# theteamatx/x-edr-trajectory-planning

Measured on AMD Instinct MI355X. Metric: time-optimal path timings/s (7-DOF, 2000 s-samples), 1/2/4/8 MI355X + %HBM roofline, higher is better.
Workload: dtype f64

## Files before the change

x-edr-trajectory-planning_amd/csrc/tpamd_sweep_joint.h:

```cpp
#pragma once

#include <type_traits>

#include "tpamd_kernels.h"

namespace tpamd {

__device__ __forceinline__ double uniform_f64(double v) {
  const int lo = __builtin_amdgcn_readfirstlane(__double2loint(v));
  const int hi = __builtin_amdgcn_readfirstlane(__double2hiint(v));
  return __hiloint2double(hi, lo);
}
__device__ __forceinline__ double readlane_f64(double v, int lane) {
  const int lo = __builtin_amdgcn_readlane(__double2loint(v), lane);
  const int hi = __builtin_amdgcn_readlane(__double2hiint(v), lane);
  return __hiloint2double(hi, lo);
}
__device__ __forceinline__ int uniform_i32(int v) { return __builtin_amdgcn_readfirstlane(v); }

template <int CTRL>
__device__ __forceinline__ double dpp_f64(double v) {
  int lo = __double2loint(v), hi = __double2hiint(v);
  lo = __builtin_amdgcn_update_dpp(0, lo, CTRL, 0xf, 0xf, true);
  hi = __builtin_amdgcn_update_dpp(0, hi, CTRL, 0xf, 0xf, true);
  return __hiloint2double(hi, lo);
}

template <bool MAX>
__device__ __forceinline__ double ext2_raw(double a, double b) {
  double r;
  if (MAX) asm("v_max_f64 %0, %1, %2" : "=v"(r) : "v"(a), "v"(b));
  else asm("v_min_f64 %0, %1, %2" : "=v"(r) : "v"(a), "v"(b));
  return r;
}

template <bool MAX>
__device__ __forceinline__ double row16_extreme(double v) {
  double o;
  o = dpp_f64<0xB1>(v);  v = ext2_raw<MAX>(o, v);
  o = dpp_f64<0x4E>(v);  v = ext2_raw<MAX>(o, v);
  o = dpp_f64<0x141>(v); v = ext2_raw<MAX>(o, v);
  o = dpp_f64<0x140>(v); v = ext2_raw<MAX>(o, v);
  return v;
}

#define TPAMD_OS_STEP(HALF, C)                                                            \
  "s_mov_b32 exec_" HALF ", %[m" #C "]\n\t"                                               \
  "v_fmac_f64_dpp %[acc], %[d], %[one] row_newbcast:" #C " row_mask:0xf bank_mask:0xf\n\t"
#define TPAMD_OS_ROW(HALF, OTHER)                                                                      \
  asm volatile("s_mov_b64 %[sv], exec\n\ts_mov_b32 exec_" OTHER ", 0\n\t"                              \
               TPAMD_OS_STEP(HALF, 0) TPAMD_OS_STEP(HALF, 1) TPAMD_OS_STEP(HALF, 2) TPAMD_OS_STEP(HALF, 3)     \
               TPAMD_OS_STEP(HALF, 4) TPAMD_OS_STEP(HALF, 5) TPAMD_OS_STEP(HALF, 6) TPAMD_OS_STEP(HALF, 7)     \
               TPAMD_OS_STEP(HALF, 8) TPAMD_OS_STEP(HALF, 9) TPAMD_OS_STEP(HALF, 10) TPAMD_OS_STEP(HALF, 11)   \
               TPAMD_OS_STEP(HALF, 12) TPAMD_OS_STEP(HALF, 13) TPAMD_OS_STEP(HALF, 14) TPAMD_OS_STEP(HALF, 15) \
               "s_mov_b64 exec, %[sv]\n\t"                                                             \
               : [acc] "+v"(acc), [sv] "=&s"(save)                                                     \
               : [d] "v"(d), [one] "v"(one), TPAMD_OS_M(0), TPAMD_OS_M(1), TPAMD_OS_M(2), TPAMD_OS_M(3), \
                 TPAMD_OS_M(4), TPAMD_OS_M(5), TPAMD_OS_M(6), TPAMD_OS_M(7), TPAMD_OS_M(8), TPAMD_OS_M(9), \
                 TPAMD_OS_M(10), TPAMD_OS_M(11), TPAMD_OS_M(12), TPAMD_OS_M(13), TPAMD_OS_M(14), TPAMD_OS_M(15))
template <int ROW>
__device__ __forceinline__ void ordered_sum_row(double &acc, double d, double one) {
  constexpr unsigned SH = (ROW & 1) ? 16u : 0u;
#define TPAMD_OS_M(C) [m##C] "n"((int)(((0xffffu << C) & 0xffffu) << SH))
  unsigned long long save;
  if (ROW < 2) TPAMD_OS_ROW("lo", "hi");
  else TPAMD_OS_ROW("hi", "lo");
#undef TPAMD_OS_M
}
template <int ROW>
__device__ __forceinline__ void ordered_sum_carry(double &acc) {
  int lo = __double2loint(acc), hi = __double2hiint(acc);
  lo = __builtin_amdgcn_update_dpp(lo, lo, 0x142, 1 << ROW, 0xf, false);
  hi = __builtin_amdgcn_update_dpp(hi, hi, 0x142, 1 << ROW, 0xf, false);
  acc = __hiloint2double(hi, lo);
}
__device__ __forceinline__ double ordered_sum64(double t, double d) {
  double acc = t;
  const double one = 1.0;
  ordered_sum_row<0>(acc, d, one);
  ordered_sum_carry<1>(acc);
  ordered_sum_row<1>(acc, d, one);
  ordered_sum_carry<2>(acc);
  ordered_sum_row<2>(acc, d, one);
  ordered_sum_carry<3>(acc);
  ordered_sum_row<3>(acc, d, one);
  return acc;
}

struct OrderedSumMasks {
  double m[15];
  __device__ __forceinline__ void init(int lane) {
#pragma unroll
    for (int c = 1; c < 16; c++) m[c - 1] = ((lane & 15) >= c) ? 1.0 : 0.0;
  }
};
#define TPAMD_OSM_STEP(C, ROWMASK)                                                                    \
  "v_fmac_f64_dpp %[acc], %[d], %[m" #C "] row_newbcast:" #C " row_mask:" ROWMASK " bank_mask:0xf\n\t"
#define TPAMD_OSM_ROW(ROWMASK)                                                                          \
  asm volatile(TPAMD_OSM_STEP(0, ROWMASK) TPAMD_OSM_STEP(1, ROWMASK) TPAMD_OSM_STEP(2, ROWMASK)         \
               TPAMD_OSM_STEP(3, ROWMASK) TPAMD_OSM_STEP(4, ROWMASK) TPAMD_OSM_STEP(5, ROWMASK)         \
               TPAMD_OSM_STEP(6, ROWMASK) TPAMD_OSM_STEP(7, ROWMASK) TPAMD_OSM_STEP(8, ROWMASK)         \
               TPAMD_OSM_STEP(9, ROWMASK) TPAMD_OSM_STEP(10, ROWMASK) TPAMD_OSM_STEP(11, ROWMASK)       \
               TPAMD_OSM_STEP(12, ROWMASK) TPAMD_OSM_STEP(13, ROWMASK) TPAMD_OSM_STEP(14, ROWMASK)      \
               TPAMD_OSM_STEP(15, ROWMASK)                                                              \
               : [acc] "+v"(acc)                                                                        \
               : [d] "v"(d), [m0] "v"(one), [m1] "v"(k.m[0]), [m2] "v"(k.m[1]), [m3] "v"(k.m[2]),       \
                 [m4] "v"(k.m[3]), [m5] "v"(k.m[4]), [m6] "v"(k.m[5]), [m7] "v"(k.m[6]), [m8] "v"(k.m[7]), \
                 [m9] "v"(k.m[8]), [m10] "v"(k.m[9]), [m11] "v"(k.m[10]), [m12] "v"(k.m[11]),           \
                 [m13] "v"(k.m[12]), [m14] "v"(k.m[13]), [m15] "v"(k.m[14]))
__device__ __forceinline__ double ordered_sum64_finite(double t, double d, const OrderedSumMasks &k) {
  double acc = t;
  const double one = 1.0;
  asm volatile("s_nop 1" ::: "memory");
  TPAMD_OSM_ROW("0x1");
  ordered_sum_carry<1>(acc);
  TPAMD_OSM_ROW("0x2");
  ordered_sum_carry<2>(acc);
  TPAMD_OSM_ROW("0x4");
  ordered_sum_carry<3>(acc);
  TPAMD_OSM_ROW("0x8");
  return acc;
}

#ifdef TPAMD_DIAG
__device__ __forceinline__ long long tpamd_stamp() {
  unsigned long long t;
  __builtin_amdgcn_sched_barrier(0);
  asm volatile("s_memtime %0\n\ts_waitcnt lgkmcnt(0)" : "=s"(t)::"memory");
  __builtin_amdgcn_sched_barrier(0);
  return (long long)t;
}
#define TPAMD_T0(var) const long long var = tpamd_stamp()
#ifdef TPAMD_DIAG_REASONS
#define TPAMD_ACC(slot, var) do { if (!((slot) == 12 || (slot) == 13 || (slot) == 17 || ((slot) >= 19 && (slot) <= 23) || (slot) == 31)) diag[slot] += tpamd_stamp() - (var); } while (0)
#else
#define TPAMD_ACC(slot, var) diag[slot] += tpamd_stamp() - (var)
#endif
#define TPAMD_CNT(slot) diag[slot] += 1
#define TPAMD_ADD(slot, v) diag[slot] += (v)
#define TPAMD_T0C(var) const long long var = tpamd_stamp()
#define TPAMD_ACCC(slot, var) diag[slot] += tpamd_stamp() - (var)
#ifdef TPAMD_DIAG_LIGHT
#undef TPAMD_T0
#undef TPAMD_ACC
#define TPAMD_T0(var)
#define TPAMD_ACC(slot, var)
#endif
#else
#define TPAMD_T0(var)
#define TPAMD_ACC(slot, var)
#define TPAMD_T0C(var)
#define TPAMD_ACCC(slot, var)
#define TPAMD_CNT(slot)
#define TPAMD_ADD(slot, v)
#endif

#ifndef TPAMD_TILE_SAMPLES
#define TPAMD_TILE_SAMPLES 32
#endif
#ifndef TPAMD_CHAIN_GUESS
#define TPAMD_CHAIN_GUESS 0
#endif
#ifndef TPAMD_CURVE_EXIT
#define TPAMD_CURVE_EXIT 1
#endif
constexpr int kTileSamples = TPAMD_TILE_SAMPLES;
template <int D>
struct TileCfg {
  static constexpr int kSamples = (D > 8 && TPAMD_TILE_SAMPLES > 16) ? 16 : TPAMD_TILE_SAMPLES;
};

typedef double f64x2 __attribute__((ext_vector_type(2)));

template <int K>
struct RegPack {
  f64x2 v;
  RegPack<K - 1> rest;
  template <int LIMIT>
  __device__ __forceinline__ void load(const f64x2 *src, int c) {
    if (c < LIMIT) v = src[c];
    rest.template load<LIMIT>(src, c + 64);
  }
  template <int LIMIT>
  __device__ __forceinline__ void store(f64x2 *dst, int c) const {
    if (c < LIMIT) dst[c] = v;
    rest.template store<LIMIT>(dst, c + 64);
  }
};
template <>
struct RegPack<0> {
  template <int LIMIT> __device__ __forceinline__ void load(const f64x2 *, int) {}
  template <int LIMIT> __device__ __forceinline__ void store(f64x2 *, int) const {}
};

template <int D>
struct JointLayout {
  static constexpr int PARTS = (D <= 7) ? 4 : ((D <= 16) ? 2 : 1);
  static constexpr int RPL = (D + PARTS - 1) / PARTS;
  static constexpr int kCandLanes = 2 * D * PARTS;
  static constexpr int kRows16 = (kCandLanes + 15) / 16;
  static_assert(kCandLanes <= 64, "candidate lanes must fit one wave");
#ifndef TPAMD_CHAIN_STEPS
#define TPAMD_CHAIN_STEPS 16
#endif
  static constexpr int kChain = TPAMD_CHAIN_STEPS;
  static constexpr int GRP = 64 / kChain;
  static constexpr int CPL = (2 * D + GRP - 1) / GRP;
  static constexpr int VPL = (D + GRP - 1) / GRP;
  static constexpr unsigned long long kPart0 =
      (GRP == 4) ? 0x1111111111111111ull : ((GRP == 2) ? 0x5555555555555555ull : ~0ull);
  static_assert(GRP == 1 || GRP == 2 || GRP == 4, "chain steps must be 16, 32 or 64");
};

template <bool MAX>
__device__ __forceinline__ double ext2(double a, double b) {
  return ext2_raw<MAX>(a, b);
}

template <int D, int E = 0>
struct JointSweep {
  typedef JointLayout<D> L;
  static_assert(E == 0 || E == 2, "extra rows come as one pair");
  static constexpr int R = 2 * D + E + 2;
  static constexpr int kMt = D + E / 2;
  static constexpr int kTile = TileCfg<D>::kSamples;
  static constexpr int kChunks = kTile * R / 2;
  static constexpr int kChunksPerLane = (kChunks + 63) / 64;
#ifdef TPAMD_DIAG
  long long diag[32];
#endif
  int N, lane;
  double ds, two_ds;
  double *sd2;
  double *tiles;
  const uint8_t *typel;
  double *sdd_g;
  const double *m_g;
  const double *rec;
  int tag0, tag1;
  double *qd_g, *qdd_g;
  const double *aml;
  uint32_t *dirty;
  int end_idx;
  double lim;
  double chk_hi[L::RPL];
  double vel_hi;
  double vel_lo;
  int vel_mode;
  double ex_hi[E ? E : 1];
  int own_off;
  int chk_off[L::RPL];
  int vel_off;
  double row_lo, row_hi;
  double v_lim[L::CPL];
  int v_off[L::CPL];
  double vv_hi[L::VPL];
  double va_hi[L::VPL];
  int vv_off[L::VPL];

  struct Rows {
    f64x2 own;
    f64x2 chk[L::RPL];
    f64x2 vel;
  };

  static __device__ __forceinline__ void wave_lds_sync() {
    __builtin_amdgcn_fence(__ATOMIC_ACQ_REL, "wavefront");
    __builtin_amdgcn_wave_barrier();
  }

  struct Prefetch {
    RegPack<kChunksPerLane> r;
    double m;
    int tag;
  };
  __device__ __forceinline__ void issue_tile_loads(int t, Prefetch &pf) const {
    const f64x2 *src = reinterpret_cast<const f64x2 *>(rec + (size_t)t * kTile * R);
    pf.r.template load<kChunks>(src, lane);
    pf.m = m_g[min(t * kTile + (lane & (kTile - 1)), N - 1)];
    pf.tag = t;
  }
  __device__ __forceinline__ void store_tile(int slot, const Prefetch &pf) const {
    f64x2 *dst = reinterpret_cast<f64x2 *>(tiles + (size_t)slot * kTile * R);
    pf.r.template store<kChunks>(dst, lane);
    wave_lds_sync();
    if (lane < kTile) {
      const int i = min(pf.tag * kTile + lane, N - 1);
      f64x2 mt;
      mt.x = pf.m;
      mt.y = __longlong_as_double((long long)typel[i]);
      dst[(size_t)lane * (R / 2) + kMt] = mt;
    }
    wave_lds_sync();
  }
  __device__ __forceinline__ void fill_tile(int t, int dir, Prefetch &pf) {
    TPAMD_T0(tf_);
    TPAMD_CNT(27);
    if (pf.tag != t) issue_tile_loads(t, pf);
    wave_lds_sync();
    store_tile(t & 1, pf);
    if (t & 1) tag1 = t; else tag0 = t;
    const int tn = t + dir;
    pf.tag = -1;
    if (tn >= 0 && tn * kTile < N) issue_tile_loads(tn, pf);
    TPAMD_ACC(28, tf_);
  }
  __device__ __forceinline__ void ensure_tile(int idx, int dir, Prefetch &pf) {
    const int t = idx / kTile;
    const int tag = (t & 1) ? tag1 : tag0;
    if (tag != t) fill_tile(t, dir, pf);
  }
  __device__ __forceinline__ const f64x2 *record(int idx) const {
    return reinterpret_cast<const f64x2 *>(tiles) + (size_t)(idx & (2 * kTile - 1)) * (R / 2);
  }
  __device__ __forceinline__ void load_rows(int idx, Rows &r) const {
    const f64x2 *p = record(idx);
    r.own = p[own_off];
#pragma unroll
    for (int k = 0; k < L::RPL; k++) r.chk[k] = p[chk_off[k]];
    r.vel = p[vel_off];
  }
  __device__ __forceinline__ void load_mt(int idx, double &m, int &t) const {
    const f64x2 v = record(idx)[kMt];
    m = v.x;
    t = __double2loint(v.y);
  }

  __device__ __forceinline__ void put_sd2(int i, double v) {
    if (lane == 0) sd2[i] = v;
    __builtin_amdgcn_wave_barrier();
  }
  __device__ __forceinline__ void put_sdd(int i, double v) {
    if (lane == 0) sdd_g[i] = v;
  }

  __device__ __forceinline__ bool emitting() const { return qd_g != nullptr || qdd_g != nullptr; }
  __device__ __forceinline__ void emit_value(int i, int d, f64x2 pr, double v, double a,
                                             double amx) const {
    const size_t o = (size_t)i * D + d;
    if (qd_g) qd_g[o] = pr.x * v;
    if (qdd_g) {
      const double v2 = v * v;
      double acc = pr.x * a + pr.y * v2;
      if (acc < -amx) acc = -amx;
      if (acc > amx) acc = amx;
      qdd_g[o] = acc;
    }
  }
  __device__ __forceinline__ int emit_range(int lo, int hi, int wv, int nwv,
                                            const volatile int *stop = nullptr,
                                            int stop_value = 0) const {
    if (!emitting() || hi < lo) return hi + 1;
    const f64x2 *rec2 = reinterpret_cast<const f64x2 *>(rec);
    for (int s0 = lo + 64 * wv; s0 <= hi; s0 += 64 * nwv) {
      if (stop != nullptr && *stop == stop_value) return s0;
      const int cnt = min(64, hi - s0 + 1);
      const int mine = s0 + min(lane, cnt - 1);
      const double s2l = sd2[mine];
      const double al = sdd_g[mine];
      const double vl = sqrt(s2l);
      constexpr int G = (D <= 8) ? D : 7;
#pragma unroll
      for (int u0 = 0; u0 < D; u0 += G) {
        f64x2 pr[G];
        double amx[G];
        int se[G];
#pragma unroll
        for (int g = 0; g < G; g++) {
          const int e = min(64 * (u0 + g) + lane, cnt * D - 1);
          se[g] = e / D;
          const int dd = e - se[g] * D;
          pr[g] = rec2[(size_t)(s0 + se[g]) * (R / 2) + dd];
          amx[g] = aml[dd];
        }
#pragma unroll
        for (int g = 0; g < G; g++) {
          if (u0 + g >= D) continue;
          const int src = se[g] << 2;
          const double v = __hiloint2double(__builtin_amdgcn_ds_bpermute(src, __double2hiint(vl)),
                                            __builtin_amdgcn_ds_bpermute(src, __double2loint(vl)));
          const double a = __hiloint2double(__builtin_amdgcn_ds_bpermute(src, __double2hiint(al)),
                                            __builtin_amdgcn_ds_bpermute(src, __double2loint(al)));
          const int e = 64 * (u0 + g) + lane;
          if (e < cnt * D) emit_value(s0 + se[g], e - se[g] * D, pr[g], v, a, amx[g]);
        }
      }
    }
    return hi + 1;
  }
  __device__ __forceinline__ void mark_dirty(int i) const {
    if (lane == 0) atomicOr(&dirty[i >> 5], 1u << (i & 31));
  }

  template <bool MAX>
  __device__ __forceinline__ double find_sdd(const Rows &r, double s2, int &win) const {
    constexpr double kSentinel = MAX ? -DBL_MAX : DBL_MAX;
    bool vel_bad;
    if (E == 0) {
      const double vv = (r.vel.x * r.vel.x) * s2;
      vel_bad = (vv + kTiny < 0.0) | (vv - kTiny > vel_hi);
    } else {
      const double sel = (vel_mode == 2) ? r.vel.y : r.vel.x;
      const double bb = (vel_mode == 0) ? sel * sel : sel;
      const double vv = bb * s2;
      vel_bad = (vv + kTiny < vel_lo) | (vv - kTiny > vel_hi);
    }
    const double sddi = (lim - r.own.y * s2) / r.own.x;
    bool bad = (fabs(r.own.x) < kTiny) | (sddi != sddi);
#pragma unroll
    for (int k = 0; k < L::RPL; k++) {
      const double v = r.chk[k].x * sddi + r.chk[k].y * s2;
      bad = bad | (fabs(v) - kTiny > chk_hi[k]);
    }
    double best = bad ? kSentinel : sddi;
    const double mine = best;
    if (L::PARTS >= 2) best = ext2<!MAX>(best, dpp_f64<0xB1>(best));
    if (L::PARTS >= 4) best = ext2<!MAX>(best, dpp_f64<0x4E>(best));
    if (L::PARTS < 2) best = ext2<MAX>(best, dpp_f64<0xB1>(best));
    if (L::PARTS < 4) best = ext2<MAX>(best, dpp_f64<0x4E>(best));
    best = ext2<MAX>(best, dpp_f64<0x141>(best));
    best = ext2<MAX>(best, dpp_f64<0x140>(best));
    double res = best;
#pragma unroll
    for (int k = 0; k < L::kRows16; k++) {
      const double rowv = readlane_f64(best, 16 * k);
      if (MAX) asm("s_nop 1\n\tv_max_f64 %0, %1, %2" : "=v"(res) : "v"(res), "s"(rowv));
      else asm("s_nop 1\n\tv_min_f64 %0, %1, %2" : "=v"(res) : "v"(res), "s"(rowv));
    }
    const unsigned long long holders = __ballot(mine == res);
    win = __ffsll((long long)holders) - 1;
    if (res == kSentinel) { res = 0; win = -1; }
    if (__ballot(vel_bad) != 0ull) { res = 0; win = -1; }
    return res;
  }

  struct ChainOperands {
    f64x2 pvv[L::VPL];
    f64x2 pown[L::CPL];
    double rc[L::CPL];
    f64x2 ex;
  };
  __device__ __forceinline__ void load_chain_operands(int j, ChainOperands &o) const {
    const f64x2 *p = record(j);
#pragma unroll
    for (int i = 0; i < L::VPL; i++) o.pvv[i] = p[vv_off[i]];
#pragma unroll
    for (int i = 0; i < L::CPL; i++) o.pown[i] = p[v_off[i]];
    if (E > 0) o.ex = p[D];
#pragma unroll
    for (int i = 0; i < L::CPL; i++) o.rc[i] = __builtin_amdgcn_rcp(o.pown[i].x);
  }
  template <bool MAX>
  __device__ __forceinline__ bool chain_step_bad(const ChainOperands &o, int win_cand, double hi_r,
                                                 f64x2 arow, double s2, double sddw, int &guess) const {
    bool bad = false;
#pragma unroll
    for (int i = 0; i < L::VPL; i++) {
      const f64x2 pr = o.pvv[i];
      const double v = pr.x * sddw + pr.y * s2;
      const bool viol = fabs(v) - kTiny > va_hi[i];
      bad = bad | viol;
      if (viol) guess = 2 * vv_off[i] + (v > 0.0 ? 1 : 0);
      const double vv = (pr.x * pr.x) * s2;
      bad = bad | (vv - kTiny > vv_hi[i]);
    }
    if (E > 0) {
      const double v0 = o.ex.x * s2, v1 = o.ex.y * s2;
      bad = bad | (fabs(v0) - kTiny > ex_hi[0]);
      bad = bad | (fabs(v1) - kTiny > ex_hi[E - 1]);
    }
    const int p0 = lane & (L::GRP - 1);
    const double better_than = MAX ? sddw - 2e-6 * fabs(sddw) : sddw + 2e-6 * fabs(sddw);
    const double row_limit = (hi_r + 2.0 * kTiny) * (1.0 + 2e-12);
    const double bs_r = arow.y * s2;
#pragma unroll
    for (int i = 0; i < L::CPL; i++) {
      const f64x2 own = o.pown[i];
      const double lim_i = v_lim[i];
      const bool skip = (lim_i != lim_i) | (fabs(own.x) < kTiny) | (p0 + L::GRP * i == win_cand);
      const double sa = (lim_i - own.y * s2) * o.rc[i];
      const bool not_better = MAX ? (__builtin_fma(2e-6, fabs(sa), sa) < better_than)
                                  : (__builtin_fma(-2e-6, fabs(sa), sa) > better_than);
      const double ax = arow.x * sa;
      const double va = ax + bs_r;
      const bool violates = __builtin_fma(-2e-6, fabs(ax), fabs(va) * (1.0 - 1e-12)) > row_limit;
      const bool beats = !(skip | not_better | violates);
      bad = bad | beats;
      if (beats) guess = p0 + L::GRP * i;
    }
    return bad;
  }

  __device__ __forceinline__ bool derivs_valid(int idx, double sddv, double s2) const {
    bool bad = false;
    if (lane < 2 * D + E) {
      const bool extra = lane >= 2 * D;
      const int d = extra ? D : ((lane < D) ? lane : lane - D);
      const f64x2 pr = record(idx)[d];
      const double A = (lane < D) ? pr.x : 0.0;
      double Bc = (lane < D) ? pr.y : pr.x * pr.x;
      if (E > 0 && extra) Bc = (lane == 2 * D) ? pr.x : pr.y;
      const double v = A * sddv + Bc * s2;
      bad = (v + kTiny < row_lo) || (v - kTiny > row_hi);
    }
    return __ballot(bad) == 0ull;
  }

  __device__ __forceinline__ void sdd_at_intersection(int index) {
    const double s2 = sd2[index];
    const bool has_next = index < N - 1, has_prev = index > 0;
    double res = 0.0;
    bool done = false;
    if (has_next && has_prev) {
      const double c = 0.25 / ds * (sd2[index + 1] - sd2[index - 1]);
      if (derivs_valid(index, c, s2)) { res = c; done = true; }
    }
    if (!done && has_next) {
      const double c = 0.5 / ds * (sd2[index + 1] - s2);
      if (derivs_valid(index, c, s2)) { res = c; done = true; }
    }
    if (!done && has_prev) {
      const double c = 0.5 / ds * (s2 - sd2[index - 1]);
      if (derivs_valid(index, c, s2)) { res = c; done = true; }
    }
    put_sdd(index, res);
    end_idx = index;
  }

  struct Carry {
    int idx;
    double cur;
    double m_i;
    double m_n;
    double nxt;
    int t_i, t_n;
    int win;
  };
  static constexpr int kContinue = -2;

  template <bool FWD>
  __device__ __forceinline__ int extremal_step(Carry &c, const Rows &use, Rows &stage, Prefetch &pf,
                                               int idx_start, bool &pair_signal, bool &pair_wait) {
    constexpr int dir = FWD ? 1 : -1;
#define TPAMD_PAIR_SIGNAL()                                   \
  do {                                                        \
    if (pair_signal) {                                        \
      __threadfence_block();                                  \
      __syncthreads();                                        \
      pair_signal = false;                                    \
    }                                                         \
  } while (0)
#define TPAMD_PAIR_WAIT()                                     \
  do {                                                        \
    if (FWD && pair_wait) {                                   \
      __syncthreads();                                        \
      pair_wait = false;                                      \
    }                                                         \
  } while (0)
    const int idx = c.idx;
    const int nidx = idx + dir;
    const bool more = FWD ? (nidx < N - 2) : (nidx > 1);
    if (((nidx + dir) & (kTile - 1)) == (FWD ? 0 : kTile - 1))
      ensure_tile(nidx + dir, dir, pf);
    load_rows(nidx, stage);
    double m_nn;
    int t_nn;
    load_mt(nidx + dir, m_nn, t_nn);
    const double nxt_nn = sd2[nidx + dir];
    const double cur = c.cur, m_i = c.m_i, m_n = c.m_n, nxt = c.nxt;
    const bool on_boundary = is_tiny(cur - m_i);
    double sd2tmp, sddtmp;
    if (on_boundary && (c.t_i & kBndTrajectory) && (c.t_n & kBndTrajectory)) {
      sd2tmp = m_n;
      sddtmp = FWD ? 0.5 * (sd2tmp - cur) / ds : 0.5 * (cur - sd2tmp) / ds;
      c.win = -1;
    } else {
      TPAMD_CNT(10);
      int win;
      sddtmp = uniform_f64(find_sdd<FWD>(use, cur, win));
      c.win = uniform_i32(win);
      sd2tmp = FWD ? cur + two_ds * sddtmp : cur - two_ds * sddtmp;
    }
    if (!isnan(nxt) && (nxt < sd2tmp)) {
      TPAMD_PAIR_WAIT();
      sdd_at_intersection(idx);
      TPAMD_PAIR_SIGNAL();
      return FWD ? N - 1 : 0;
    }
    if (sd2tmp > m_n) {
      const double sdd_bound = FWD ? 0.5 * (m_n - cur) / ds : 0.5 * (cur - m_n) / ds;
      const bool deriv_invalid = !derivs_valid(idx, sdd_bound, FWD ? m_i : cur);
      const bool type_invalid = c.t_n & (FWD ? kBndSink : kBndSource);
      const bool stop = FWD ? (type_invalid || deriv_invalid)
                            : ((type_invalid || deriv_invalid) && !(idx_start != (N - 1)));
      if (stop) {
        end_idx = idx;
        TPAMD_PAIR_SIGNAL();
        TPAMD_PAIR_WAIT();
        return idx;
      }
      sd2tmp = m_n;
      sddtmp = sdd_bound;
      c.win = -1;
    }
    if (sd2tmp < 0) {
      TPAMD_PAIR_WAIT();
      c.win = -1;
      sd2tmp = 0.0;
      if (FWD) {
        if (idx <= 1) sddtmp = 0.0; else sddtmp = -sd2[idx - 1] / ds;
      } else {
        if (idx < N - 1) sddtmp = sd2[idx + 1] / ds; else sddtmp = 0.0;
      }
    }
    TPAMD_PAIR_WAIT();
    put_sd2(nidx, sd2tmp);
    put_sdd(idx, sddtmp);
    if (!more) end_idx = nidx;
    TPAMD_PAIR_SIGNAL();
    if (!more) return FWD ? N - 1 : 0;
    c.idx = nidx;
    c.cur = sd2tmp;
    c.m_i = m_n;
    c.t_i = c.t_n;
    c.m_n = uniform_f64(m_nn);
    c.t_n = uniform_i32(t_nn);
    c.nxt = uniform_f64(nxt_nn);
    return kContinue;
#undef TPAMD_PAIR_SIGNAL
#undef TPAMD_PAIR_WAIT
  }

  template <bool FWD>
  __device__ __forceinline__ int follow_boundary(Carry &c) {
    constexpr int dir = FWD ? 1 : -1;
    const int j = c.idx + dir * lane;
    const bool in_loop = FWD ? (j < N - 2) : (j > 1);
    bool elig = false;
    double m_jn = 0.0, m_j = 0.0;
    const int jn = j + dir;
    const int tj = max(j, 0) / kTile, tjn = max(jn, 0) / kTile;
    const bool resident = (tj == tag0 || tj == tag1) && (tjn == tag0 || tjn == tag1);
    if (in_loop && j >= 0 && j < N && resident) {
      const f64x2 mt_j = record(j)[kMt], mt_n = record(jn)[kMt];
      m_j = mt_j.x;
      m_jn = mt_n.x;
      const double nxt = sd2[jn];
      elig = (__double2loint(mt_j.y) & kBndTrajectory) && (__double2loint(mt_n.y) & kBndTrajectory) &&
             !(!isnan(nxt) && (nxt < m_jn)) && !(m_jn < 0);
    }
    const unsigned long long mask = __ballot(elig);
    const int L = (~mask == 0ull) ? 64 : (__ffsll((long long)~mask) - 1);
    if (L == 0) return 0;
    const double cur_k = (lane == 0) ? c.cur : m_j;
    const double sddv = FWD ? 0.5 * (m_jn - cur_k) / ds : 0.5 * (cur_k - m_jn) / ds;
    if (lane < L) {
      sd2[j + dir] = m_jn;
      sdd_g[j] = sddv;
    }
    wave_lds_sync();
    c.idx += dir * L;
    c.cur = readlane_f64(m_jn, L - 1);
    return L;
  }

  template <bool FWD>
  __device__ __forceinline__ int follow_chain(Carry &c, Prefetch &pf, int &next_win, bool &curve) {
    constexpr int dir = FWD ? 1 : -1;
    constexpr int K = L::kChain;
    next_win = -1;
    curve = false;
    const int wl = c.win;
    const int r = (wl / L::PARTS) >> 1;
    const double alim = readlane_f64(lim, wl);
    const int j0 = c.idx;
    int jl = j0 + dir * K;
    jl = FWD ? min(jl, N - 1) : max(jl, 0);
    ensure_tile(j0, dir, pf);
    ensure_tile(jl, dir, pf);
    constexpr int G = L::GRP;
    const int k = lane / G;
    int j = j0 + dir * k;
    const bool in_loop = FWD ? (j < N - 2) : (j > 1);
    j = min(max(j, 0), N - 1);
    const int jn = min(max(j + dir, 0), N - 1);
    const f64x2 arow = record(j)[r];
    const double hi_r = readlane_f64(row_hi, r);
    ChainOperands ops;
    load_chain_operands(j, ops);
    const f64x2 mt_j = record(j)[kMt], mt_n = record(jn)[kMt];
    const double nxt = sd2[jn];
    double y = __builtin_amdgcn_rcp(arow.x);
    {
      double e = __builtin_fma(-arow.x, y, 1.0);
      y = __builtin_fma(y, e, y);
      e = __builtin_fma(-arow.x, y, 1.0);
      y = __builtin_fma(y, e, y);
    }
    static_assert(G == 4 && K == 16, "the lane pipeline below assumes four lanes per step and 16-lane DPP rows");
    double x = c.cur, y_out = 0.0;
#pragma unroll
    for (int s = 0; s < K; s++) {
      const double n = alim - arow.y * x;
      const double q0 = n * y;
      const double rem = __builtin_fma(-arow.x, q0, n);
      const double q = __builtin_fma(rem, y, q0);
      y_out = FWD ? x + two_ds * q : x - two_ds * q;
      if (s + 1 < K) {
        int lo = __double2loint(x), hi = __double2hiint(x);
        const int ylo = __double2loint(y_out), yhi = __double2hiint(y_out);
        lo = __builtin_amdgcn_update_dpp(lo, ylo, 0x114, 0xf, 0xf, false);
        hi = __builtin_amdgcn_update_dpp(hi, yhi, 0x114, 0xf, 0xf, false);
        if ((s & 3) == 3) {
          lo = __builtin_amdgcn_update_dpp(lo, ylo, 0x142, 0xe, 0x1, false);
          hi = __builtin_amdgcn_update_dpp(hi, yhi, 0x142, 0xe, 0x1, false);
        }
        x = __hiloint2double(hi, lo);
      }
    }
    const double my_cur = x;
    const double my_sdd = (alim - arow.y * my_cur) / arow.x;
    const double my_new = FWD ? my_cur + two_ds * my_sdd : my_cur - two_ds * my_sdd;
    const double chain_next = y_out;
    const bool bits_equal = __double_as_longlong(chain_next) == __double_as_longlong(my_new);
    int guess = -1;
    const bool bad = chain_step_bad<FWD>(ops, wl / L::PARTS, hi_r, arow, my_cur, my_sdd, guess) |
                     is_tiny(arow.x);
    const int t_j = __double2loint(mt_j.y), t_n = __double2loint(mt_n.y);
    const double m_j = mt_j.x, m_n = mt_n.x;
    const bool riding = is_tiny(my_cur - m_j) & ((t_j & kBndTrajectory) != 0) & ((t_n & kBndTrajectory) != 0);
    const bool special = riding | (!isnan(nxt) & (nxt < my_new)) | (my_new < 0) | isnan(my_new);
    const unsigned long long fo = __ballot(bad | !in_loop | !bits_equal | special);
    unsigned long long fm = fo | __ballot(my_new > m_n);
    if (G >= 2) fm |= fm >> 1;
    if (G >= 4) fm |= fm >> 2;
    const unsigned long long miss = fm & L::kPart0;
    const int Lc = miss ? ((__ffsll((long long)miss) - 1) / G) : K;
#ifdef TPAMD_DIAG_REASONS
    if (Lc < K) {
      const unsigned long long lanes_ = ((1ull << G) - 1ull) << (G * Lc);
      const bool r_loop = (__ballot(!in_loop) & lanes_) != 0, r_eq = (__ballot(!bits_equal) & lanes_) != 0;
      const bool r_ride = (__ballot(riding) & lanes_) != 0, r_isect = (__ballot(!isnan(nxt) & (nxt < my_new)) & lanes_) != 0;
      const bool r_curve = (__ballot(my_new > m_n) & lanes_) != 0, r_neg = (__ballot((my_new < 0) | isnan(my_new)) & lanes_) != 0;
      const bool r_bad = (__ballot(bad) & lanes_) != 0, r_hint = (__ballot(guess >= 0) & lanes_) != 0;
      if (r_loop) diag[19]++; else if (r_ride) diag[20]++; else if (r_isect) diag[21]++; else if (r_curve) diag[22]++;
      else if (r_neg) diag[23]++; else if (r_eq) diag[31]++; else if (r_bad && r_hint) diag[13]++; else if (r_bad) diag[12]++;
      if (Lc == 0) diag[17]++;
    }
#endif
    if (TPAMD_CHAIN_GUESS && Lc > 0 && Lc < K) {
      const unsigned long long other = __ballot(!in_loop | !bits_equal | special | (my_new > m_n));
      const unsigned long long hints = __ballot(guess >= 0);
      const unsigned long long lanes = ((1ull << G) - 1ull) << (G * Lc);
      if ((other & lanes) == 0ull && (hints & lanes) != 0ull) {
        const int src = __ffsll((long long)(hints & lanes)) - 1;
        next_win = __builtin_amdgcn_readlane(guess, src) * L::PARTS;
      }
    }
    if (TPAMD_CURVE_EXIT && Lc < K) {
      const unsigned long long lanes = ((1ull << G) - 1ull) << (G * Lc);
      if ((fo & lanes) == 0ull) {
        curve = true;
        c.m_i = readlane_f64(m_j, G * Lc);
        c.m_n = readlane_f64(m_n, G * Lc);
        c.t_n = __builtin_amdgcn_readlane(t_n, G * Lc);
      }
    }
    if (Lc == 0) return 0;
    if ((lane & (G - 1)) == 0 && k < Lc) {
      sd2[j + dir] = my_new;
      sdd_g[j] = my_sdd;
    }
    wave_lds_sync();
    c.idx = j0 + dir * Lc;
    c.cur = readlane_f64(my_new, G * (Lc - 1));
    return Lc;
  }

  template <bool FWD>
  __device__ __forceinline__ int leave_on_curve(Carry &c, int idx_start) {
    constexpr int dir = FWD ? 1 : -1;
    const int idx = c.idx, nidx = idx + dir;
    const bool more = FWD ? (nidx < N - 2) : (nidx > 1);
    const double cur = c.cur, m_n = c.m_n;
    const double sdd_bound = FWD ? 0.5 * (m_n - cur) / ds : 0.5 * (cur - m_n) / ds;
    const bool deriv_invalid = !derivs_valid(idx, sdd_bound, FWD ? c.m_i : cur);
    const bool type_invalid = c.t_n & (FWD ? kBndSink : kBndSource);
    const bool stop = FWD ? (type_invalid || deriv_invalid)
                          : ((type_invalid || deriv_invalid) && !(idx_start != (N - 1)));
    if (stop) {
      end_idx = idx;
      return idx;
    }
    double sd2tmp = m_n, sddtmp = sdd_bound;
    c.win = -1;
    if (sd2tmp < 0) {
      sd2tmp = 0.0;
      if (FWD) {
        if (idx <= 1) sddtmp = 0.0; else sddtmp = -sd2[idx - 1] / ds;
      } else {
        if (idx < N - 1) sddtmp = sd2[idx + 1] / ds; else sddtmp = 0.0;
      }
    }
    put_sd2(nidx, sd2tmp);
    put_sdd(idx, sddtmp);
    if (!more) {
      end_idx = nidx;
      return FWD ? N - 1 : 0;
    }
    c.idx = nidx;
    c.cur = sd2tmp;
    return kContinue;
  }

  template <bool FWD>
  __device__ __forceinline__ void init_carry(int idx, Carry &c, Rows &rows, Prefetch &pf, bool load_cur) {
    constexpr int dir = FWD ? 1 : -1;
    TPAMD_T0(ti_);
    TPAMD_CNT(29);
    c.idx = idx;
    ensure_tile(idx, dir, pf);
    ensure_tile(idx + dir, dir, pf);
    load_rows(idx, rows);
    if (load_cur) c.cur = uniform_f64(sd2[idx]);
    double m0, m1;
    int t0, t1;
    load_mt(idx, m0, t0);
    load_mt(idx + dir, m1, t1);
    c.m_i = uniform_f64(m0); c.m_n = uniform_f64(m1);
    c.t_i = uniform_i32(t0); c.t_n = uniform_i32(t1);
    c.nxt = uniform_f64(sd2[idx + dir]);
    c.win = -1;
    TPAMD_ACC(26, ti_);
  }

  template <bool FWD>
  __device__ __forceinline__ int add_extremal(int idx_start, Prefetch &pf, bool pair_signal = false,
                                              bool wait_pair = false) {
#define TPAMD_PAIR_SIGNAL()                                   \
  do {                                                        \
    if (pair_signal) {                                        \
      __threadfence_block();                                  \
      __syncthreads();                                        \
      pair_signal = false;                                    \
    }                                                         \
  } while (0)
    if (FWD ? !(idx_start < N - 2) : !(idx_start > 1)) {
      end_idx = idx_start;
      TPAMD_PAIR_SIGNAL();
      if (wait_pair) __syncthreads();
      return FWD ? N - 1 : 0;
    }
    Rows rows_a, rows_b;
    Carry c;
    init_carry<FWD>(idx_start, c, rows_a, pf, true);
    if (wait_pair && is_tiny(c.cur - c.m_i) && (c.t_i & kBndTrajectory) && (c.t_n & kBndTrajectory)) {
      __syncthreads();
      wait_pair = false;
    }
    bool trust = true;
    int last_win = -1;
    for (;;) {
#define TPAMD_TRY_FOLLOW()                                                                   \
  if (is_tiny(c.cur - c.m_i) && (c.t_i & kBndTrajectory) && (c.t_n & kBndTrajectory)) {      \
    TPAMD_T0(tfb_);                                                                          \
    const int run = uniform_i32(follow_boundary<FWD>(c));                                    \
    TPAMD_ACC(25, tfb_);                                                                     \
    if (run > 0) {                                                                           \
      TPAMD_CNT(8);                                                                          \
      TPAMD_PAIR_SIGNAL();                                                                   \
      if (FWD ? !(c.idx < N - 2) : !(c.idx > 1)) {                                           \
        end_idx = c.idx;                                                                     \
        return FWD ? N - 1 : 0;                                                              \
      }                                                                                      \
      init_carry<FWD>(c.idx, c, rows_a, pf, false);                                          \
      continue;                                                                              \
    }                                                                                        \
  }
#define TPAMD_TRY_CHAIN()                                                                    \
  if (c.win >= 0 && (trust || c.win == last_win)) {                                          \
    int total = 0, run, next_win;                                                            \
    bool again, curve;                                                                       \
    do {                                                                                     \
      { TPAMD_T0(tc_); run = uniform_i32(follow_chain<FWD>(c, pf, next_win, curve)); TPAMD_ACC(4, tc_); } \
      TPAMD_CNT(6);                                                                          \
      total += run;                                                                          \
      again = run == L::kChain;                                                              \
       \
      if (run > 0 && run < L::kChain && next_win >= 0) { c.win = uniform_i32(next_win); again = true; } \
    } while (again && (FWD ? (c.idx < N - 2) : (c.idx > 1)));                                \
    trust = total > 0;                                                                       \
    last_win = -1;                                                                           \
    TPAMD_ADD(14, total);                                                                    \
    if (curve) {                                                                             \
       \
      TPAMD_CNT(30);                                                                         \
      trust = true;                                                                          \
      const int rc = leave_on_curve<FWD>(c, idx_start);                                      \
      if (rc != kContinue) return rc;                                                        \
      total = 1;          \
    }                                                                                        \
    if (total > 0) {                                                                         \
      if (FWD ? !(c.idx < N - 2) : !(c.idx > 1)) {                                           \
        end_idx = c.idx;                                                                     \
        return FWD ? N - 1 : 0;                                                              \
      }                                                                                      \
      init_carry<FWD>(c.idx, c, rows_a, pf, false);                                          \
      continue;                                                                              \
    }                                                                                        \
  } else {                                                                                   \
    last_win = c.win;                                                                        \
  }
      TPAMD_TRY_FOLLOW();
      TPAMD_T0(ts1_);
      int r = extremal_step<FWD>(c, rows_a, rows_b, pf, idx_start, pair_signal, wait_pair);
      TPAMD_ACC(24, ts1_);
      if (r != kContinue) return r;
      TPAMD_TRY_CHAIN();
      if (is_tiny(c.cur - c.m_i) && (c.t_i & kBndTrajectory) && (c.t_n & kBndTrajectory)) {
        load_rows(c.idx, rows_a);
        continue;
      }
      TPAMD_T0(ts2_);
      r = extremal_step<FWD>(c, rows_b, rows_a, pf, idx_start, pair_signal, wait_pair);
      TPAMD_ACC(24, ts2_);
      if (r != kContinue) return r;
      TPAMD_TRY_CHAIN();
    }
#undef TPAMD_TRY_CHAIN
#undef TPAMD_TRY_FOLLOW
#undef TPAMD_PAIR_SIGNAL
  }

  __device__ __forceinline__ int next_critical_point(int idx_lo, int idx_hi, int zlast) const {
    int c0 = -1;
    for (int base = idx_lo + 1; base <= idx_hi && c0 < 0; base += 256) {
      uint8_t ty[4];
#pragma unroll
      for (int u = 0; u < 4; u++) ty[u] = typel[min(base + 64 * u + lane, N - 1)];
      unsigned long long mask[4];
#pragma unroll
      for (int u = 0; u < 4; u++) {
        const int idx = base + 64 * u + lane;
        mask[u] = __ballot((idx <= idx_hi) & ((ty[u] & (kBndSource | kBndTrajectory)) != 0));
      }
#pragma unroll
      for (int u = 3; u >= 0; u--)
        if (mask[u]) c0 = base + 64 * u + __ffsll((long long)mask[u]) - 1;
    }
    if (c0 < 0) return -1;
    return (zlast > c0) ? zlast : c0;
  }

  __device__ __forceinline__ int last_flagged_below(int idx_hi) const {
    for (int top = idx_hi; top >= 1; top -= 256) {
      uint8_t ty[4];
#pragma unroll
      for (int u = 0; u < 4; u++) ty[u] = typel[max(top - 64 * u - lane, 0)];
#pragma unroll
      for (int u = 0; u < 4; u++) {
        const int idx = top - 64 * u - lane;
        const unsigned long long m = __ballot((idx >= 1) & ((ty[u] & kBndEqualsZ00) != 0));
        if (m) return top - 64 * u - (__ffsll((long long)m) - 1);
      }
    }
    return -1;
  }

#ifdef TPAMD_DIAG
  __device__ __forceinline__ int next_critical_point_literal(int idx_lo, int idx_hi) const {
    int crit = -1;
    for (int idx = idx_lo + 1; idx <= idx_hi; idx++) {
      if (crit < 0) {
        if (typel[idx] & (kBndSource | kBndTrajectory)) crit = idx;
      } else if (typel[idx] & kBndEqualsZ00) {
        crit = idx;
      }
      if (crit > 0 && !isnan(sd2[idx])) return crit;
    }
    return -1;
  }
#endif
};

constexpr int kRefitCap = 128;
constexpr int kRefitLdsBytes = kRefitCap * (4 + 8 + 8);

template <int D, int E>
struct PathBoundary {
  const JointSource &src;
  const Workspace &ws;
  int b, N, stride, lane;
  size_t pb;
  double ds, z00;
  const uint8_t *at_l;
  uint8_t *ff_l, *typel;
  bool keep;
  int *l_idx;
  double *l_val, *l_nxt;
  int count;

  __device__ __forceinline__ void append(bool need, int j, double val, double nxt) {
    const unsigned long long mask = __ballot(need);
    if (!mask) return;
    if (need) {
      const int pos = count + __popcll(mask & ((1ull << lane) - 1ull));
      l_idx[pos] = j;
      l_val[pos] = val;
      l_nxt[pos] = nxt;
    }
    count += __popcll(mask);
  }

  __device__ __forceinline__ void refit_one(int j, double sd2v, double *x, double *y) const {
    constexpr int R = 2 * D + E + 2;
    const f64x2 *rec2 = reinterpret_cast<const f64x2 *>(src.q12 + ((size_t)b * stride + j) * R);
    const double *lim_lo = src.lim + (size_t)b * 2 * (2 * D + E), *lim_hi = lim_lo + 2 * D + E;
    double a[D], bq[D];
#pragma unroll
    for (int d = 0; d < D; d++) {
      const f64x2 p = rec2[d];
      a[d] = p.x;
      bq[d] = p.y;
    }
    bool ok = true;
    if (E > 0) {
      const f64x2 ex = rec2[D];
      const double vt = ex.x * sd2v, vr = ex.y * sd2v;
      ok = !(vt + kTiny < lim_lo[2 * D] || vt - kTiny > lim_hi[2 * D]) &&
           !(vr + kTiny < lim_lo[2 * D + 1] || vr - kTiny > lim_hi[2 * D + 1]);
    }
    if (ok) find_sdd_both_joint_fixed<D>(a, bq, lim_hi, sd2v, x, y);
  }

  __device__ __forceinline__ void finalize(int j, double m, double X, double Y, double m_next) const {
    uint8_t type = kBndNone;
    if (j >= 1 && j <= N - 2) {
      const double sd2p = (m_next - m) / ds;
      const double sd2p_min = 2 * Y;
      const double sd2p_max = 2 * X;
      if (sd2p < sd2p_min) type = kBndSink;
      else if (sd2p > sd2p_max) type = kBndSource;
      if ((sd2p <= sd2p_max) && (sd2p >= sd2p_min)) type = kBndTrajectory;
    }
    if (m == z00) type |= kBndEqualsZ00;
    ws.m[pb + j] = m;
    typel[j] = type;
    if (keep) {
      ws.X[pb + j] = X;
      ws.Y[pb + j] = Y;
      ws.type[pb + j] = type;
    }
  }

  template <bool FINAL>
  __device__ __forceinline__ void flush(long long *diag) {
    TPAMD_T0(tf);
    __builtin_amdgcn_fence(__ATOMIC_ACQ_REL, "wavefront");
    __builtin_amdgcn_wave_barrier();
    const int n = count;
    for (int e = lane; e < n; e += 64) {
      const int j = l_idx[e];
      const double val = l_val[e];
      double x = 0.0, y = 0.0;
      refit_one(j, val, &x, &y);
      if (FINAL) finalize(j, val, x, y, l_nxt[e]);
      else { ws.Xz[pb + j] = x; ws.Yz[pb + j] = y; }
    }
    count = 0;
    __builtin_amdgcn_fence(__ATOMIC_ACQ_REL, "wavefront");
    __builtin_amdgcn_wave_barrier();
    if (FINAL) TPAMD_ACC(23, tf);
  }
};

template <int D, int E>
__device__ __forceinline__ void boundary_passes_for_path(const JointSource &src, const Workspace &ws, int b,
                                                         int N, int stride, int tid, uint8_t *at_l,
                                                         uint8_t *ff_l, char *scratch, uint8_t *typel,
                                                         bool keep, long long *diag) {
  TPAMD_T0C(tp0);
// ... 969 lines not shown
```

Baseline: 2.131 million.

## Exit chain-following early on intersection and support truncated chain rounds

Adds an intersection-exit path in the chain follower: when the first failing lane is caused only by the chain crossing the previously computed curve, the sweep breaks out and resolves the intersection directly via sdd_at_intersection instead of falling back to extremal stepping. It also adds an optional CHAIN_CUT mode, off by default, that stops the 16-step DPP pipeline early, and makes the continue condition depend on whether all computed rounds succeeded. The intent is to skip wasted extremal steps near intersections. The risk is a changed control flow for the sweep termination, which has to match the existing intersection semantics.

```diff
diff --git a/x-edr-trajectory-planning_amd/csrc/tpamd_sweep_joint.h b/x-edr-trajectory-planning_amd/csrc/tpamd_sweep_joint.h
--- a/x-edr-trajectory-planning_amd/csrc/tpamd_sweep_joint.h
+++ b/x-edr-trajectory-planning_amd/csrc/tpamd_sweep_joint.h
@@ -132,7 +132,7 @@
 }
 #define TPAMD_T0(var) const long long var = tpamd_stamp()
 #ifdef TPAMD_DIAG_REASONS
-#define TPAMD_ACC(slot, var) do { if (!((slot) == 12 || (slot) == 13 || (slot) == 17 || ((slot) >= 19 && (slot) <= 23) || (slot) == 31)) diag[slot] += tpamd_stamp() - (var); } while (0)
+#define TPAMD_ACC(slot, var) do { if (!((slot) == 2 || (slot) == 4 || (slot) == 12 || (slot) == 13 || (slot) == 16 || (slot) == 17 || ((slot) >= 19 && (slot) <= 26) || (slot) == 28 || (slot) == 31)) diag[slot] += tpamd_stamp() - (var); } while (0)
 #else
 #define TPAMD_ACC(slot, var) diag[slot] += tpamd_stamp() - (var)
 #endif
@@ -163,6 +163,12 @@
 #endif
 #ifndef TPAMD_CURVE_EXIT
 #define TPAMD_CURVE_EXIT 1
+#endif
+#ifndef TPAMD_ISECT_EXIT
+#define TPAMD_ISECT_EXIT 1
+#endif
+#ifndef TPAMD_CHAIN_CUT
+#define TPAMD_CHAIN_CUT 0
 #endif
 constexpr int kTileSamples = TPAMD_TILE_SAMPLES;
 template <int D>
@@ -665,11 +671,13 @@
   }
 
   template <bool FWD>
-  __device__ __forceinline__ int follow_chain(Carry &c, Prefetch &pf, int &next_win, bool &curve) {
+  __device__ __forceinline__ int follow_chain(Carry &c, Prefetch &pf, int &next_win, bool &curve, bool &isect,
+                                              bool &full) {
     constexpr int dir = FWD ? 1 : -1;
     constexpr int K = L::kChain;
     next_win = -1;
     curve = false;
+    isect = false;
     const int wl = c.win;
     const int r = (wl / L::PARTS) >> 1;
     const double alim = readlane_f64(lim, wl);
@@ -698,6 +706,8 @@
       y = __builtin_fma(y, e, y);
     }
     static_assert(G == 4 && K == 16, "the lane pipeline below assumes four lanes per step and 16-lane DPP rows");
+    const int n_in = FWD ? (N - 2 - j0) : (j0 - 1);
+    int rounds = K;
     double x = c.cur, y_out = 0.0;
 #pragma unroll
     for (int s = 0; s < K; s++) {
@@ -706,6 +716,19 @@
       const double rem = __builtin_fma(-arow.x, q0, n);
       const double q = __builtin_fma(rem, y, q0);
       y_out = FWD ? x + two_ds * q : x - two_ds * q;
+      if (TPAMD_CHAIN_CUT && (s & 3) == 3 && s + 1 < K) {
+        bool stop;
+        if (TPAMD_CHAIN_CUT == 2) {
+          stop = s / 4 == ((j0 >> 2) & 3);
+        } else {
+          const unsigned long long kFinal = (1ull << (16 * (s / 4 + 1))) - 1ull;
+          stop = (s + 1 >= n_in) || (__ballot((y_out > mt_n.x) | (nxt < y_out)) & kFinal) != 0ull;
+        }
+        if (stop) {
+          rounds = s + 1;
+          break;
+        }
+      }
       if (s + 1 < K) {
         int lo = __double2loint(x), hi = __double2hiint(x);
         const int ylo = __double2loint(y_out), yhi = __double2hiint(y_out);
@@ -719,6 +742,7 @@
       }
     }
     const double my_cur = x;
+    const bool run = in_loop & (k < rounds);
     const double my_sdd = (alim - arow.y * my_cur) / arow.x;
     const double my_new = FWD ? my_cur + two_ds * my_sdd : my_cur - two_ds * my_sdd;
     const double chain_next = y_out;
@@ -730,7 +754,7 @@
     const double m_j = mt_j.x, m_n = mt_n.x;
     const bool riding = is_tiny(my_cur - m_j) & ((t_j & kBndTrajectory) != 0) & ((t_n & kBndTrajectory) != 0);
     const bool special = riding | (!isnan(nxt) & (nxt < my_new)) | (my_new < 0) | isnan(my_new);
-    const unsigned long long fo = __ballot(bad | !in_loop | !bits_equal | special);
+    const unsigned long long fo = __ballot(bad | !run | !bits_equal | special);
     unsigned long long fm = fo | __ballot(my_new > m_n);
     if (G >= 2) fm |= fm >> 1;
     if (G >= 4) fm |= fm >> 2;
@@ -739,7 +763,7 @@
 #ifdef TPAMD_DIAG_REASONS
     if (Lc < K) {
       const unsigned long long lanes_ = ((1ull << G) - 1ull) << (G * Lc);
-      const bool r_loop = (__ballot(!in_loop) & lanes_) != 0, r_eq = (__ballot(!bits_equal) & lanes_) != 0;
+      const bool r_loop = (__ballot(!run) & lanes_) != 0, r_eq = (__ballot(!bits_equal) & lanes_) != 0;
       const bool r_ride = (__ballot(riding) & lanes_) != 0, r_isect = (__ballot(!isnan(nxt) & (nxt < my_new)) & lanes_) != 0;
       const bool r_curve = (__ballot(my_new > m_n) & lanes_) != 0, r_neg = (__ballot((my_new < 0) | isnan(my_new)) & lanes_) != 0;
       const bool r_bad = (__ballot(bad) & lanes_) != 0, r_hint = (__ballot(guess >= 0) & lanes_) != 0;
@@ -747,9 +771,14 @@
       else if (r_neg) diag[23]++; else if (r_eq) diag[31]++; else if (r_bad && r_hint) diag[13]++; else if (r_bad) diag[12]++;
       if (Lc == 0) diag[17]++;
     }
+    {
+      const int shape = rounds / 4 - 1;
+      diag[shape == 0 ? 24 : (shape == 1 ? 25 : (shape == 2 ? 26 : 28))]++;
+      if (shape < 3) diag[shape == 0 ? 2 : (shape == 1 ? 4 : 16)] += Lc;
+    }
 #endif
     if (TPAMD_CHAIN_GUESS && Lc > 0 && Lc < K) {
-      const unsigned long long other = __ballot(!in_loop | !bits_equal | special | (my_new > m_n));
+      const unsigned long long other = __ballot(!run | !bits_equal | special | (my_new > m_n));
       const unsigned long long hints = __ballot(guess >= 0);
       const unsigned long long lanes = ((1ull << G) - 1ull) << (G * Lc);
       if ((other & lanes) == 0ull && (hints & lanes) != 0ull) {
@@ -757,15 +786,20 @@
         next_win = __builtin_amdgcn_readlane(guess, src) * L::PARTS;
       }
     }
-    if (TPAMD_CURVE_EXIT && Lc < K) {
+    if ((TPAMD_CURVE_EXIT || TPAMD_ISECT_EXIT) && Lc < K) {
       const unsigned long long lanes = ((1ull << G) - 1ull) << (G * Lc);
-      if ((fo & lanes) == 0ull) {
+      if (TPAMD_CURVE_EXIT && (fo & lanes) == 0ull) {
         curve = true;
         c.m_i = readlane_f64(m_j, G * Lc);
         c.m_n = readlane_f64(m_n, G * Lc);
         c.t_n = __builtin_amdgcn_readlane(t_n, G * Lc);
       }
-    }
+      if (TPAMD_ISECT_EXIT && (fo & lanes) != 0ull &&
+          (__ballot(bad | !run | !bits_equal | riding) & lanes) == 0ull &&
+          (__ballot(nxt < my_new) & lanes) != 0ull)
+        isect = true;
+    }
+    full = Lc == rounds;
     if (Lc == 0) return 0;
     if ((lane & (G - 1)) == 0 && k < Lc) {
       sd2[j + dir] = my_new;
@@ -880,18 +914,20 @@
 #define TPAMD_TRY_CHAIN()                                                                    \
   if (c.win >= 0 && (trust || c.win == last_win)) {                                          \
     int total = 0, run, next_win;                                                            \
-    bool again, curve;                                                                       \
+    bool again, curve, isect, full;                                                          \
     do {                                                                                     \
-      { TPAMD_T0(tc_); run = uniform_i32(follow_chain<FWD>(c, pf, next_win, curve)); TPAMD_ACC(4, tc_); } \
+      { TPAMD_T0(tc_); run = uniform_i32(follow_chain<FWD>(c, pf, next_win, curve, isect, full)); TPAMD_ACC(4, tc_); } \
       TPAMD_CNT(6);                                                                          \
       total += run;                                                                          \
-      again = run == L::kChain;                                                              \
+      again = full;                                                                          \
        \
       if (run > 0 && run < L::kChain && next_win >= 0) { c.win = uniform_i32(next_win); again = true; } \
     } while (again && (FWD ? (c.idx < N - 2) : (c.idx > 1)));                                \
     trust = total > 0;                                                                       \
     last_win = -1;                                                                           \
     TPAMD_ADD(14, total);                                                                    \
+     \
+    if (isect) break;                                                                        \
     if (curve) {                                                                             \
        \
       TPAMD_CNT(30);                                                                         \
@@ -927,6 +963,9 @@
       if (r != kContinue) return r;
       TPAMD_TRY_CHAIN();
     }
+    TPAMD_CNT(30);
+    sdd_at_intersection(c.idx);
+    return FWD ? N - 1 : 0;
 #undef TPAMD_TRY_CHAIN
 #undef TPAMD_TRY_FOLLOW
 #undef TPAMD_PAIR_SIGNAL
```

New measurement: 2.124 million (median of 3 runs). About the same (-0.3%).

## Hand over boundary-follow state to carry init and use permlane swaps for reductions

Applied to the files above, without the earlier changes.

Replaces the serial readlane/s_nop min-max loop across 16-lane rows with permlane16/permlane32 swap reductions. When follow_boundary or the chain step has already loaded the next index's m, t and sd2 values, it stores them in the Carry with a held flag. init_carry then skips tile checks and reloads. This shortens the latency-bound serial sweep. The risk is stale handed-over values if tile residency or state changes between the handover and the next step.

```diff
diff --git a/x-edr-trajectory-planning_amd/csrc/tpamd_sweep_joint.h b/x-edr-trajectory-planning_amd/csrc/tpamd_sweep_joint.h
--- a/x-edr-trajectory-planning_amd/csrc/tpamd_sweep_joint.h
+++ b/x-edr-trajectory-planning_amd/csrc/tpamd_sweep_joint.h
@@ -42,6 +42,21 @@
   o = dpp_f64<0x141>(v); v = ext2_raw<MAX>(o, v);
   o = dpp_f64<0x140>(v); v = ext2_raw<MAX>(o, v);
   return v;
+}
+
+template <bool MAX>
+__device__ __forceinline__ double row_swap_extreme(double v) {
+  const unsigned lo = (unsigned)__double2loint(v), hi = (unsigned)__double2hiint(v);
+  const auto l = __builtin_amdgcn_permlane16_swap(lo, lo, false, false);
+  const auto h = __builtin_amdgcn_permlane16_swap(hi, hi, false, false);
+  return ext2_raw<MAX>(__hiloint2double((int)h[0], (int)l[0]), __hiloint2double((int)h[1], (int)l[1]));
+}
+template <bool MAX>
+__device__ __forceinline__ double half_swap_extreme(double v) {
+  const unsigned lo = (unsigned)__double2loint(v), hi = (unsigned)__double2hiint(v);
+  const auto l = __builtin_amdgcn_permlane32_swap(lo, lo, false, false);
+  const auto h = __builtin_amdgcn_permlane32_swap(hi, hi, false, false);
+  return ext2_raw<MAX>(__hiloint2double((int)h[0], (int)l[0]), __hiloint2double((int)h[1], (int)l[1]));
 }
 
 #define TPAMD_OS_STEP(HALF, C)                                                            \
@@ -161,6 +176,9 @@
 #ifndef TPAMD_CHAIN_GUESS
 #define TPAMD_CHAIN_GUESS 0
 #endif
+#ifndef TPAMD_HANDOVER
+#define TPAMD_HANDOVER 1
+#endif
 #ifndef TPAMD_CURVE_EXIT
 #define TPAMD_CURVE_EXIT 1
 #endif
@@ -420,13 +438,8 @@
     if (L::PARTS < 4) best = ext2<MAX>(best, dpp_f64<0x4E>(best));
     best = ext2<MAX>(best, dpp_f64<0x141>(best));
     best = ext2<MAX>(best, dpp_f64<0x140>(best));
-    double res = best;
-#pragma unroll
-    for (int k = 0; k < L::kRows16; k++) {
-      const double rowv = readlane_f64(best, 16 * k);
-      if (MAX) asm("s_nop 1\n\tv_max_f64 %0, %1, %2" : "=v"(res) : "v"(res), "s"(rowv));
-      else asm("s_nop 1\n\tv_min_f64 %0, %1, %2" : "=v"(res) : "v"(res), "s"(rowv));
-    }
+    double res = (L::kRows16 > 2) ? half_swap_extreme<MAX>(row_swap_extreme<MAX>(best))
+                       : (L::kRows16 > 1) ? row_swap_extreme<MAX>(best) : best;
     const unsigned long long holders = __ballot(mine == res);
     win = __ffsll((long long)holders) - 1;
     if (res == kSentinel) { res = 0; win = -1; }
@@ -535,6 +548,7 @@
     double nxt;
     int t_i, t_n;
     int win;
+    bool held;
   };
   static constexpr int kContinue = -2;
 
@@ -637,16 +651,19 @@
     const int j = c.idx + dir * lane;
     const bool in_loop = FWD ? (j < N - 2) : (j > 1);
     bool elig = false;
-    double m_jn = 0.0, m_j = 0.0;
+    double m_jn = 0.0, m_j = 0.0, nxt = 0.0;
+    int t_jn = 0;
     const int jn = j + dir;
     const int tj = max(j, 0) / kTile, tjn = max(jn, 0) / kTile;
     const bool resident = (tj == tag0 || tj == tag1) && (tjn == tag0 || tjn == tag1);
-    if (in_loop && j >= 0 && j < N && resident) {
+    const bool loaded = in_loop && j >= 0 && j < N && resident;
+    if (loaded) {
       const f64x2 mt_j = record(j)[kMt], mt_n = record(jn)[kMt];
       m_j = mt_j.x;
       m_jn = mt_n.x;
-      const double nxt = sd2[jn];
-      elig = (__double2loint(mt_j.y) & kBndTrajectory) && (__double2loint(mt_n.y) & kBndTrajectory) &&
+      t_jn = __double2loint(mt_n.y);
+      nxt = sd2[jn];
+      elig = (__double2loint(mt_j.y) & kBndTrajectory) && (t_jn & kBndTrajectory) &&
              !(!isnan(nxt) && (nxt < m_jn)) && !(m_jn < 0);
     }
     const unsigned long long mask = __ballot(elig);
@@ -661,6 +678,14 @@
     wave_lds_sync();
     c.idx += dir * L;
     c.cur = readlane_f64(m_jn, L - 1);
+    c.held = L < 64 && ((__ballot(loaded) >> L) & 1ull);
+    if (c.held) {
+      c.m_i = c.cur;
+      c.t_i = __builtin_amdgcn_readlane(t_jn, L - 1);
+      c.m_n = readlane_f64(m_jn, L);
+      c.t_n = __builtin_amdgcn_readlane(t_jn, L);
+      c.nxt = readlane_f64(nxt, L);
+    }
     return L;
   }
 
@@ -757,13 +782,19 @@
         next_win = __builtin_amdgcn_readlane(guess, src) * L::PARTS;
       }
     }
+    c.held = Lc < K;
+    if (Lc < K) {
+      c.m_i = readlane_f64(m_j, G * Lc);
+      c.m_n = readlane_f64(m_n, G * Lc);
+      c.t_i = __builtin_amdgcn_readlane(t_j, G * Lc);
+      c.t_n = __builtin_amdgcn_readlane(t_n, G * Lc);
+      c.nxt = readlane_f64(nxt, G * Lc);
+    }
     if (TPAMD_CURVE_EXIT && Lc < K) {
       const unsigned long long lanes = ((1ull << G) - 1ull) << (G * Lc);
       if ((fo & lanes) == 0ull) {
         curve = true;
-        c.m_i = readlane_f64(m_j, G * Lc);
-        c.m_n = readlane_f64(m_n, G * Lc);
-        c.t_n = __builtin_amdgcn_readlane(t_n, G * Lc);
+        c.held = false;
       }
     }
     if (Lc == 0) return 0;
@@ -818,19 +849,25 @@
     constexpr int dir = FWD ? 1 : -1;
     TPAMD_T0(ti_);
     TPAMD_CNT(29);
+    const bool held = TPAMD_HANDOVER && c.held;
     c.idx = idx;
-    ensure_tile(idx, dir, pf);
-    ensure_tile(idx + dir, dir, pf);
+    if (!held) {
+      ensure_tile(idx, dir, pf);
+      ensure_tile(idx + dir, dir, pf);
+    }
     load_rows(idx, rows);
     if (load_cur) c.cur = uniform_f64(sd2[idx]);
-    double m0, m1;
-    int t0, t1;
-    load_mt(idx, m0, t0);
-    load_mt(idx + dir, m1, t1);
-    c.m_i = uniform_f64(m0); c.m_n = uniform_f64(m1);
-    c.t_i = uniform_i32(t0); c.t_n = uniform_i32(t1);
-    c.nxt = uniform_f64(sd2[idx + dir]);
+    if (!held) {
+      double m0, m1;
+      int t0, t1;
+      load_mt(idx, m0, t0);
+      load_mt(idx + dir, m1, t1);
+      c.m_i = uniform_f64(m0); c.m_n = uniform_f64(m1);
+      c.t_i = uniform_i32(t0); c.t_n = uniform_i32(t1);
+      c.nxt = uniform_f64(sd2[idx + dir]);
+    }
     c.win = -1;
+    c.held = false;
     TPAMD_ACC(26, ti_);
   }
 
@@ -853,6 +890,7 @@
     }
     Rows rows_a, rows_b;
     Carry c;
+    c.held = false;
     init_carry<FWD>(idx_start, c, rows_a, pf, true);
     if (wait_pair && is_tiny(c.cur - c.m_i) && (c.t_i & kBndTrajectory) && (c.t_n & kBndTrajectory)) {
       __syncthreads();
```

Result: no change. 2.111 million before, 2.109 million after (median of 4 runs) (-0.1%).
